# ivanalberico/End-To-End-Self-Supervised-SLAM

Hardware: AMD Instinct MI355X
Metric: online refinement steps/sec @640x480, seq_len=60 (higher is better)
Workload: dtype f32

## Files before the change

### end-to-end-self-supervised-slam_amd/csrc/conv.hip

```cpp
#include <cassert>
#include <type_traits>

#include "e2e_common.h"

typedef float f4v __attribute__((ext_vector_type(4)));
typedef float f16v __attribute__((ext_vector_type(16)));

#define CBK 16

enum { ACT_NONE = 0, ACT_RELU = 1, ACT_ELU = 2, ACT_DISP = 3 };

struct ConvArgs {
    const float* src0;
    const float* src1;
    const float* w;
    const float* scale;
    const float* shift;
    const float* res;
    float* out;
    int B, Hs, Ws;
    int Cin, C1, up;
    int Hd, Wd;
    int Ncols, ldw;
    int KH, KW, stride, pad, pad_mode;
// ... 794 lines not shown
#pragma unroll
            for (int q = 0; q < 4; ++q) {
                const f4v t = {v[4 * q], v[4 * q + 1], v[4 * q + 2], v[4 * q + 3]};
                __builtin_amdgcn_raw_buffer_store_b128(__builtin_bit_cast(__attribute__((__vector_size__(4 * sizeof(unsigned)))) unsigned, t), rsl, sl_off + q * 64 * 16, 0, SK_SC1);
            }
            asm volatile("s_waitcnt vmcnt(0)" ::: "memory");
            __syncthreads();
            if (tid == 0) __hip_atomic_store(&s.flags[g], 1u, __ATOMIC_RELAXED, __HIP_MEMORY_SCOPE_AGENT);
        } else {
            if (ce != s.C) {
                const int64_t tile_end = (int64_t)(tile + 1) * s.C;
                int h_last = g;
                for (int h = g + 1; h < s.G && s.I * h / s.G < tile_end; ++h) h_last = h;
                if (tid == 0) {
                    for (int h = g + 1; h <= h_last; ++h) {
                        unsigned spins = 0;
                        while (__hip_atomic_load(&s.flags[h], __ATOMIC_RELAXED, __HIP_MEMORY_SCOPE_AGENT) == 0u) {
                            __builtin_amdgcn_s_sleep(2);
                            if (++spins > (1u << 24)) { __hip_atomic_store(&s.flags[SK_ERR_INDEX], 1u, __ATOMIC_RELAXED, __HIP_MEMORY_SCOPE_AGENT); break; }
                        }
                    }
                    __builtin_amdgcn_fence(__ATOMIC_ACQUIRE, "agent");
                }
                asm volatile("s_waitcnt vmcnt(0)" ::: "memory");
                __syncthreads();
                for (int h = g + 1; h <= h_last; ++h) {
                    const __amdgpu_buffer_rsrc_t rsl = __builtin_amdgcn_make_buffer_rsrc((void*)(s.slabs + (int64_t)h * (BM * BN)), 0, BM * BN * 4, 0x00020000);
                    f4v t[4];
#pragma unroll
                    for (int q = 0; q < 4; ++q) t[q] = __builtin_bit_cast(f4v, __builtin_amdgcn_raw_buffer_load_b128(rsl, sl_off + q * 64 * 16, 0, SK_SC1));
#pragma unroll
                    for (int q = 0; q < 4; ++q)
#pragma unroll
                        for (int e = 0; e < 4; ++e) acc[4 * q + e] += t[q][e];
                }
                if (tid == 0)
                    for (int h = g + 1; h <= h_last; ++h) __hip_atomic_store(&s.flags[h], 0u, __ATOMIC_RELAXED, __HIP_MEMORY_SCOPE_AGENT);
            }
            const EpiRsrc er = make_epi_rsrc<TRANSPOSED>(a);
            epilogue_block<TRANSPOSED>(a, er, acc, c0 + wn * 32 + (lane & 31), n0 + wm * 32 + 4 * khalf, Ntot);
        }
        it += ce - cb;
    }
}

struct ThinArgs {
    const float* src;
    const float* w;
    const float* bias;
    float* out;
    int B, Hsrc, Wsrc, Hd, Wd, ldw, act, org, flip;
};

template <int CIN, int UP, bool REFLECT, int TH>
__global__ __launch_bounds__(256) void k_conv3x3_thin(ThinArgs a) {
    constexpr int TW = 64, PH = TH + 2, PW = TW + 2, PWS = 72, PLANE = PH * PWS, KQ = CIN / 4;
    static_assert(PLANE % 32 == 16, "the two channel planes a half-wave reads must sit 16 banks apart");
    __shared__ float patch[CIN * PLANE];
    const int tid = threadIdx.x, lane = tid & 63, wave = tid >> 6, l16 = lane & 15, kq = lane >> 4;
    const int x0 = blockIdx.x * TW, y0 = blockIdx.y * TH, b = blockIdx.z;
    const int HD = a.Hsrc * UP, WD = a.Wsrc * UP;
    float wreg[9][KQ];
#pragma unroll
    for (int t = 0; t < 9; ++t)
#pragma unroll
        for (int j = 0; j < KQ; ++j) wreg[t][j] = a.w[(int64_t)((a.flip ? 8 - t : t) * CIN + 4 * j + kq) * a.ldw + l16];
    const float* sb = a.src + (int64_t)b * a.Hsrc * a.Wsrc * CIN;
    for (int idx = tid; idx < PH * PW * KQ; idx += 256) {
        const int q = (UP == 2) ? idx / (PH * PW) : idx % KQ, pix = (UP == 2) ? idx % (PH * PW) : idx / KQ;
        const int py = pix / PW, px = pix - py * PW;
        int Y = y0 - a.org + py, X = x0 - a.org + px;
        bool ok = true;
        if (REFLECT) {
            Y = min(max(reflect1(Y, HD), 0), HD - 1);
            X = min(max(reflect1(X, WD), 0), WD - 1);
        } else {
            ok = Y >= 0 && Y < HD && X >= 0 && X < WD;
        }
        f4v v = {0.f, 0.f, 0.f, 0.f};
        if (ok) v = *(const f4v*)(sb + ((int64_t)(Y / UP) * a.Wsrc + (X / UP)) * CIN + q * 4);
#pragma unroll
        for (int e = 0; e < 4; ++e) patch[(q * 4 + e) * PLANE + py * PWS + px] = v[e];
    }
    __syncthreads();
    const float bv = a.bias ? a.bias[l16] : 0.f;
    float* ob = a.out + (int64_t)b * a.Hd * a.Wd * 16;
#pragma unroll 1
    for (int g2 = 0; g2 < TH; g2 += 2) {
        const int g0 = wave * TH + g2, g1 = g0 + 1;
        const int r0 = g0 >> 2, c0 = (g0 & 3) * 16, r1 = g1 >> 2, c1 = (g1 & 3) * 16;
        f4v acc0 = {0.f, 0.f, 0.f, 0.f}, acc1 = {0.f, 0.f, 0.f, 0.f};
        const float* p0 = patch + kq * PLANE + r0 * PWS + c0 + l16;
        const float* p1 = patch + kq * PLANE + r1 * PWS + c1 + l16;
#pragma unroll
        for (int t = 0; t < 9; ++t) {
            const int off = (t / 3) * PWS + (t % 3);
#pragma unroll
            for (int j = 0; j < KQ; ++j) {
                acc0 = __builtin_amdgcn_mfma_f32_16x16x4f32(p0[4 * j * PLANE + off], wreg[t][j], acc0, 0, 0, 0);
                acc1 = __builtin_amdgcn_mfma_f32_16x16x4f32(p1[4 * j * PLANE + off], wreg[t][j], acc1, 0, 0, 0);
            }
        }
#pragma unroll
        for (int h = 0; h < 2; ++h) {
            const f4v acc = h ? acc1 : acc0;
            const int y = y0 + (h ? r1 : r0), xb = x0 + (h ? c1 : c0) + 4 * kq;
            if (y >= a.Hd) continue;
#pragma unroll
            for (int i = 0; i < 4; ++i)
                if (xb + i < a.Wd) ob[((int64_t)y * a.Wd + xb + i) * 16 + l16] = apply_act(acc[i] + bv, a.act);
        }
    }
}

struct StemArgs {
    const float* src;
    const float* w;
    const float* scale;
    const float* shift;
    float* out;
    int B, Hs, Ws, Hd, Wd, ldw, act;
    float in_sub, in_mul;
};

__global__ __launch_bounds__(256) void k_conv7x7_stem(StemArgs a) {
    constexpr int TH = 4, TW = 32, PH = 2 * TH + 6, PW = 2 * TW + 5, ROW = 208, NJ = 37;
    __shared__ float patch[PH * ROW];
    const int tid = threadIdx.x, lane = tid & 63, wave = tid >> 6, l16 = lane & 15, kq = lane >> 4;
    const int x0 = blockIdx.x * TW, y0 = blockIdx.y * TH, b = blockIdx.z;
    const int co = 16 * wave + l16;
    float wreg[NJ];
    int offk[NJ];
#pragma unroll
    for (int j = 0; j < NJ; ++j) {
        const int k = 4 * j + kq;
        wreg[j] = k < 147 ? a.w[(int64_t)k * a.ldw + co] : 0.f;
        offk[j] = k + (k / 21) * (ROW - 21);
    }
    const float* sb = a.src + (int64_t)b * a.Hs * a.Ws * 3;
    for (int idx = tid; idx < PH * ROW; idx += 256) {
        const int py = idx / ROW, e = idx - py * ROW;
        const int Y = 2 * y0 - 3 + py, X = 2 * x0 - 3 + e / 3;
        const bool ok = e < 3 * PW && Y >= 0 && Y < a.Hs && X >= 0 && X < a.Ws;
        patch[idx] = ok ? (sb[((int64_t)Y * a.Ws + X) * 3 + (e - (e / 3) * 3)] - a.in_sub) * a.in_mul : 0.f;
    }
    __syncthreads();
    const float sc = a.scale ? a.scale[co] : 1.f, sh = a.shift ? a.shift[co] : 0.f;
    float* ob = a.out + (int64_t)b * a.Hd * a.Wd * 64;
#pragma unroll 1
    for (int g = 0; g < 2 * TH; g += 2) {
        const int r = g >> 1;
        const float* p0 = patch + 2 * r * ROW + 6 * l16;
        const float* p1 = p0 + 6 * 16;
        f4v acc0 = {0.f, 0.f, 0.f, 0.f}, acc1 = {0.f, 0.f, 0.f, 0.f};
#pragma unroll
        for (int j = 0; j < NJ; ++j) {
            acc0 = __builtin_amdgcn_mfma_f32_16x16x4f32(p0[offk[j]], wreg[j], acc0, 0, 0, 0);
            acc1 = __builtin_amdgcn_mfma_f32_16x16x4f32(p1[offk[j]], wreg[j], acc1, 0, 0, 0);
        }
        const int y = y0 + r;
        if (y >= a.Hd) continue;
#pragma unroll
        for (int h = 0; h < 2; ++h) {
            const f4v acc = h ? acc1 : acc0;
            const int xb = x0 + 16 * h + 4 * kq;
// ... 903 lines not shown
    __shared__ float dzs[TH * TW * 64];
    const int tid = threadIdx.x, lane = tid & 63, wave = tid >> 6, l16 = lane & 15, kq = lane >> 4;
    const int y0 = blockIdx.y * TH, b = blockIdx.z;
    int offn[10];
#pragma unroll
    for (int nt = 0; nt < 10; ++nt) {
        const int k = 16 * nt + l16;
        offn[nt] = k + (k / 21) * (ROW - 21) + 48 * kq;
    }
    f4v acc[10];
#pragma unroll
    for (int nt = 0; nt < 10; ++nt) acc[nt] = (f4v){0.f, 0.f, 0.f, 0.f};
    const float* sb = a.src + (int64_t)b * a.Hs * a.Ws * 3;
    const float* zb = a.dz + (int64_t)b * a.Hd * a.Wd * 64;
    for (int tx = 0; tx < a.tiles_x; ++tx) {
        const int x0 = (blockIdx.x * a.tiles_x + tx) * TW;
        if (x0 >= a.Wd) break;
        __syncthreads();
        for (int idx = tid; idx < PH * ROW; idx += 256) {
            const int py = idx / ROW, e = idx - py * ROW;
            const int Y = 2 * y0 - 3 + py, X = 2 * x0 - 3 + e / 3;
            const bool ok = e < 3 * PW && Y >= 0 && Y < a.Hs && X >= 0 && X < a.Ws;
            patch[idx] = ok ? (sb[((int64_t)Y * a.Ws + X) * 3 + (e - (e / 3) * 3)] - a.in_sub) * a.in_mul : 0.f;
        }
        for (int idx = tid; idx < TH * TW * 16; idx += 256) {
            const int q = idx & 15, pix = idx >> 4;
            const int r = pix / TW, x = pix - r * TW;
            const bool ok = y0 + r < a.Hd && x0 + x < a.Wd;
            *(f4v*)&dzs[pix * 64 + q * 4] = ok ? *(const f4v*)(zb + ((int64_t)(y0 + r) * a.Wd + x0 + x) * 64 + q * 4) : (f4v){0.f, 0.f, 0.f, 0.f};
        }
        __syncthreads();
#pragma unroll 1
        for (int r = 0; r < TH; ++r) {
            const float* ap = dzs + (r * TW + 8 * kq) * 64 + 16 * wave + l16;
            const float* bp = patch + 2 * r * ROW;
#pragma unroll 2
            for (int ks = 0; ks < TW / 4; ++ks) {
                const float av = ap[ks * 64];
#pragma unroll
                for (int nt = 0; nt < 10; ++nt) acc[nt] = __builtin_amdgcn_mfma_f32_16x16x4f32(av, bp[offn[nt] + ks * 6], acc[nt], 0, 0, 0);
            }
        }
    }
    float* slab = a.slabs + (((int64_t)b * gridDim.y + blockIdx.y) * a.nxg + blockIdx.x) * 64 * NPAD;
#pragma unroll
    for (int nt = 0; nt < 10; ++nt)
#pragma unroll
        for (int i = 0; i < 4; ++i) {
            const int n = 16 * nt + l16;
            if (n < 147) slab[(16 * wave + 4 * kq + i) * NPAD + n] = acc[nt][i];
        }
}

struct TapWgradArgs {
    const float* dz;
    const float* src0;
    const float* src1;
    float* slabs;
    int B, H, W, Cin, C1, up, Cout, reflect, has_bias, Mpad, Npad;
    int ptx, pty;
    int nchunks, cps;
};

#define TAP_NT 192
template <bool BIAS>
__global__ __launch_bounds__(TAP_NT) void k_wgrad3x3_taps(TapWgradArgs a) {
    __shared__ float dzs[64 * 32];
    __shared__ float xs[100 * 32];
    const int tid = threadIdx.x, lane = tid & 63, wave = tid >> 6, kh_ = lane >> 5, l32 = lane & 31;
    const int ci0 = blockIdx.x * 32, co0 = blockIdx.y * 32;
    const bool first = ci0 < a.C1;
    const int sh = first ? (a.up >> 1) : 0, Cs = first ? a.C1 : a.Cin - a.C1, cs0 = first ? ci0 : ci0 - a.C1;
    const int Hs = a.H >> sh, Ws = a.W >> sh;
    const float* sbase = first ? a.src0 : a.src1;
    const int c_begin = blockIdx.z * a.cps, c_end = min(c_begin + a.cps, a.nchunks);
    const bool want_bias = BIAS && blockIdx.x == 0 && wave == 0;
    f16v acc[3], accb;
#pragma unroll
    for (int t = 0; t < 3; ++t)
#pragma unroll
        for (int r = 0; r < 16; ++r) acc[t][r] = 0.f;
#pragma unroll
    for (int r = 0; r < 16; ++r) accb[r] = 0.f;
    const float one = (l32 == 0) ? 1.f : 0.f;
    f4v rz[3], rx[5];
    auto load_chunk = [&](int g) {
        const int b = g / (a.pty * a.ptx), rem = g - b * (a.pty * a.ptx), py = rem / a.ptx, px = rem - py * a.ptx;
        const int y0 = py * 8, x0 = px * 8;
        const float* zb = a.dz + (int64_t)b * a.H * a.W * a.Cout + co0;
        const float* sb = sbase + (int64_t)b * Hs * Ws * Cs + cs0;
#pragma unroll
        for (int i = 0; i < 3; ++i) {
            const int f = tid + TAP_NT * i, pix = f >> 3, q = f & 7, y = y0 + (pix >> 3), x = x0 + (pix & 7);
            const bool ok = f < 512 && y < a.H && x < a.W;
            rz[i] = ok ? *(const f4v*)(zb + ((int64_t)y * a.W + x) * a.Cout + q * 4) : (f4v){0.f, 0.f, 0.f, 0.f};
        }
#pragma unroll
        for (int i = 0; i < 5; ++i) {
            const int f = tid + TAP_NT * i;
            f4v v = {0.f, 0.f, 0.f, 0.f};
            if (f < 800) {
                const int pix = f >> 3, q = f & 7;
                int y = y0 - 1 + pix / 10, x = x0 - 1 + pix % 10;
                bool ok = true;
                if (a.reflect) {
                    y = min(max(reflect1(y, a.H), 0), a.H - 1);
// ... 857 lines not shown
    return E2E_OK;
}

struct ConvGeom { int B, Hs, Ws, Cin, Cout, Ho, Wo, KH, KW, stride, pad, pad_mode, C1, up; float in_sub, in_mul; };
#define GEOM_LAYER(g) ConvGeom g{}; g.B = B; g.Hs = Hs; g.Ws = Ws; g.Cin = Cin; g.Cout = Cout; g.KH = KH; g.KW = KW; g.stride = stride; g.pad = pad; g.pad_mode = pad_mode
#define GEOM_SOURCES(g) g.C1 = C1; g.up = up; g.in_sub = in_sub; g.in_mul = in_mul
#define GEOM_OUTPUT(g) g.Ho = Ho; g.Wo = Wo
#define GEOM_BWD_DATA(g) GEOM_LAYER(g); GEOM_OUTPUT(g)
#define GEOM_BWD_WEIGHT(g) GEOM_LAYER(g); GEOM_OUTPUT(g); GEOM_SOURCES(g)
#define GEOM_WGRAD_QUERY(g) ConvGeom g{}; g.B = B; g.Ho = Ho; g.Wo = Wo; g.Cin = Cin; g.Cout = Cout; g.KH = KH; g.KW = KW
struct FwdOps { const float *src0, *src1, *w_fwd; int ld_fwd; const float *scale, *shift, *residual; float* out; int act; };
struct BwdDataOps { const float* dz; const float* w_bwd; int ld_bwd; float* dxp; int accumulate; const float* x_in; int in_act; const float* pre_add; };
struct WgradIn { const float *dz, *src0, *src1; float* workspace; };

static int fwd_setup(const FwdOps& f, const ConvGeom& g, ConvArgs& a_out, int& vec_out, const char* who) {
    const int B = g.B, Hs = g.Hs, Ws = g.Ws, Cin = g.Cin, Cout = g.Cout, KH = g.KH, KW = g.KW, stride = g.stride, pad = g.pad, pad_mode = g.pad_mode;
    const int C1 = g.C1, up = g.up, ld_fwd = f.ld_fwd;
    E2E_REQUIRE(f.src0 && f.w_fwd && f.out && B > 0 && Hs > 0 && Ws > 0 && Cin > 0 && Cout > 0 && KH > 0 && KW > 0, E2E_ERR_ARG, "%s: bad argument", who);
    E2E_REQUIRE(up == 1 || up == 2, E2E_ERR_ARG, "%s: upsample factor must be 1 or 2", who);
    E2E_REQUIRE(C1 > 0 && C1 <= Cin && (C1 == Cin || f.src1), E2E_ERR_ARG, "%s: bad channel split", who);
    E2E_REQUIRE(pad_mode == 0 || (pad_mode == 1 && pad == 1 && Hs >= 2 && Ws >= 2), E2E_ERR_ARG, "%s: reflection padding needs pad == 1", who);
    E2E_REQUIRE(stride == 1 || stride == 2, E2E_ERR_ARG, "%s: stride must be 1 or 2", who);
    E2E_REQUIRE(Hs % up == 0 && Ws % up == 0 && ld_fwd % 4 == 0 && ld_fwd >= Cout, E2E_ERR_ARG, "%s: bad sizes", who);
    E2E_REQUIRE(pad >= 0 && Hs + 2 * pad >= KH && Ws + 2 * pad >= KW, E2E_ERR_ARG, "%s: the kernel must fit the padded input (pad >= 0)", who);
    const int vec = (Cin % 16 == 0 && (C1 == Cin || C1 % 16 == 0)) ? 4 : 1;
    E2E_REQUIRE(vec == 4 || (C1 == Cin && up == 1), E2E_ERR_ARG, "%s: the scalar path (Cin %% 16 != 0) takes a single full-resolution source", who);
    E2E_REQUIRE((int64_t)B * Hs * Ws * Cin * 4 < (1ll << 30) && (int64_t)KH * KW * Cin * ld_fwd * 4 < (1ll << 31), E2E_ERR_ARG,
                "%s: activations must stay below 1 GB, weights below 2 GB (32-bit buffer offsets with out-of-range markers)", who);
    E2E_REQUIRE(vec != 4 || (KH <= 3 && KW <= 3), E2E_ERR_ARG, "%s: the channel-quad loader takes kernels up to 3 x 3", who);
    ConvArgs a{};
    a.src0 = f.src0; a.src1 = f.src1; a.w = f.w_fwd; a.scale = f.scale; a.shift = f.shift; a.res = f.residual; a.out = f.out;
    a.B = B; a.Hs = Hs; a.Ws = Ws; a.Cin = Cin; a.C1 = C1; a.up = up;
    a.Hd = (Hs + 2 * pad - KH) / stride + 1; a.Wd = (Ws + 2 * pad - KW) / stride + 1;
    a.Ncols = Cout; a.ldw = ld_fwd; a.KH = KH; a.KW = KW; a.stride = stride; a.pad = pad; a.pad_mode = pad_mode; a.off = 0; a.act = f.act;
    a.in_sub = g.in_sub; a.in_mul = g.in_mul;
    a_out = a; vec_out = vec;
    return E2E_OK;
}

static int conv_fwd_impl(const FwdOps& f, const ConvGeom& g, float* workspace, GemmCfg force, void* stream) {
    const int B = g.B, Hs = g.Hs, Ws = g.Ws, Cin = g.Cin, Cout = g.Cout, KH = g.KH, KW = g.KW, stride = g.stride, pad = g.pad, pad_mode = g.pad_mode;
    const int C1 = g.C1, up = g.up, ld_fwd = f.ld_fwd;
    ConvArgs a;
    int vec;
    const int rc = fwd_setup(f, g, a, vec, "e2e_conv2d_fwd");
    if (rc != E2E_OK) return rc;
    if (!force.bm && KH == 7 && KW == 7 && stride == 2 && pad == 3 && pad_mode == 0 && Cin == 3 && Cout == 64 && C1 == Cin && up == 1 && !f.residual && ld_fwd >= 64) {
        StemArgs t{f.src0, f.w_fwd, f.scale, f.shift, f.out, B, Hs, Ws, a.Hd, a.Wd, ld_fwd, f.act, g.in_sub, g.in_mul};
        hipLaunchKernelGGL(k_conv7x7_stem, dim3((a.Wd + 31) / 32, (a.Hd + 3) / 4, B), dim3(256), 0, (hipStream_t)stream, t);
    }
    else if (!force.bm && KH == 3 && KW == 3 && stride == 1 && pad == 1 && pad_mode == 1 && Cout == 16 && C1 == Cin && !f.scale && !f.residual && ld_fwd >= 16 &&
        ((Cin == 16 && up == 2) || (Cin == 32 && up == 1))) {
        ThinArgs t{f.src0, f.w_fwd, f.shift, f.out, B, Hs / up, Ws / up, Hs, Ws, ld_fwd, f.act, 1, 0};
        if (Cin == 16) hipLaunchKernelGGL((k_conv3x3_thin<16, 2, true, 8>), dim3((Ws + 63) / 64, (Hs + 7) / 8, B), dim3(256), 0, (hipStream_t)stream, t);
        else hipLaunchKernelGGL((k_conv3x3_thin<32, 1, true, 4>), dim3((Ws + 63) / 64, (Hs + 3) / 4, B), dim3(256), 0, (hipStream_t)stream, t);
    } else
        launch_gemm<false>(a, vec, workspace, force, (hipStream_t)stream);
    E2E_LAUNCH_CHECK("e2e_conv2d_fwd");
    return E2E_OK;
}

int e2e_conv2d_fwd(const float* src0, const float* src1, int C1, int up, const float* w_fwd, int ld_fwd, const float* scale,
                   const float* shift, const float* residual, float* out, int B, int Hs, int Ws, int Cin, int Cout, int KH,
                   int KW, int stride, int pad, int pad_mode, int act, float in_sub, float in_mul, float* workspace, void* stream) {
    GEOM_LAYER(g); GEOM_SOURCES(g);
    return conv_fwd_impl(FwdOps{src0, src1, w_fwd, ld_fwd, scale, shift, residual, out, act}, g, workspace, GemmCfg{0, 0, 0}, stream);
}

static bool tuning_ok(int tile_m, int tile_n, int ksplit) {
    if (tile_m == 0) return true;
    if (ksplit < 0) return tile_m == 64 && tile_n == 64 && -ksplit <= SK_MAX_G;
    return tile_max_cb(tile_m, tile_n) != 0 && ksplit >= 1 && ksplit <= 16;
}

int e2e_conv2d_fwd_tuned(const float* src0, const float* src1, int C1, int up, const float* w_fwd, int ld_fwd, const float* scale,
                         const float* shift, const float* residual, float* out, int B, int Hs, int Ws, int Cin, int Cout, int KH,
                         int KW, int stride, int pad, int pad_mode, int act, float in_sub, float in_mul, float* workspace, int tile_m, int tile_n,
                         int ksplit, void* stream) {
    E2E_REQUIRE(tuning_ok(tile_m, tile_n, ksplit), E2E_ERR_ARG, "e2e_conv2d_fwd_tuned: unsupported decomposition %d x %d / %d", tile_m, tile_n, ksplit);
    GEOM_LAYER(g); GEOM_SOURCES(g);
    return conv_fwd_impl(FwdOps{src0, src1, w_fwd, ld_fwd, scale, shift, residual, out, act}, g, workspace, GemmCfg{tile_m, tile_n, ksplit}, stream);
}

struct EntryOps {
    const float* x;
    const float *w1_fwd; int ld1; const float *scale1, *shift1; float* out1; int act1; float* workspace1;
    const float* wd_fwd; int ldd; const float *gamma, *beta, *mean, *var; float eps; float *bn_scale, *bn_shift, *bn_rstd, *z, *y;
};
struct EntryPlan { ConvArgs a1, ad; int vec1, vecd; GemmLaunch p1, pd; ConvGeom g1, gd; bool paired; };

static int fwd_entry_plan(const EntryOps& q, const ConvGeom& g, EntryPlan& P, const char* who) {
    E2E_REQUIRE(q.gamma && q.beta && q.mean && q.var && q.bn_scale && q.bn_shift && q.bn_rstd && q.z && q.y, E2E_ERR_ARG, "%s: bad argument", who);
    E2E_REQUIRE(g.pad_mode == 0 && g.C1 == g.Cin && g.up == 1, E2E_ERR_ARG, "%s: a stage entry reads one zero-padded full-resolution source", who);
    P.g1 = g;
    P.gd = g; P.gd.KH = P.gd.KW = 1; P.gd.pad = 0;
    int rc = fwd_setup(FwdOps{q.x, nullptr, q.w1_fwd, q.ld1, q.scale1, q.shift1, nullptr, q.out1, q.act1}, P.g1, P.a1, P.vec1, who);
    if (rc != E2E_OK) return rc;
    rc = fwd_setup(FwdOps{q.x, nullptr, q.wd_fwd, q.ldd, nullptr, nullptr, nullptr, q.z, ACT_NONE}, P.gd, P.ad, P.vecd, who);
    if (rc != E2E_OK) return rc;
    E2E_REQUIRE(P.a1.Hd == P.ad.Hd && P.a1.Wd == P.ad.Wd, E2E_ERR_ARG, "%s: the two branches must produce the same output grid", who);
    P.paired = false;
    if (P.vec1 != 4 || P.vecd != 4 || g.Cout < 128) return E2E_OK;
    P.p1 = plan_gemm<false>(P.a1, 4, q.workspace1, GemmCfg{0, 0, 0});
    P.pd = plan_gemm<false>(P.ad, 4, nullptr, GemmCfg{0, 0, 0});
    auto t14 = [](const GemmLaunch& p) { return p.kind == GK_TILE && p.cb == 32 && p.c.bm == 32 && p.c.bn == 128; };
    P.paired = t14(P.p1) && t14(P.pd) && P.pd.tail == GT_NONE && P.ad.ksplit == 1 && P.pd.g.z == 1;
    return E2E_OK;
}
// ... 5 lines not shown
    const int pad_mode = 0, C1 = Cin, up = 1;
    const float in_sub = 0.f, in_mul = 1.f;
    GEOM_LAYER(g); GEOM_SOURCES(g);
    const EntryOps q{x, w1_fwd, ld1, scale1, shift1, out1, act1, workspace1, wd_fwd, ldd, gamma, beta, running_mean, running_var, eps, bn_scale, bn_shift, bn_rstd, z, y};
    EntryPlan P;
    int rc = fwd_entry_plan(q, g, P, "e2e_conv2d_fwd_entry_pair");
    if (rc != E2E_OK) return rc;
    const hipStream_t st = (hipStream_t)stream;
    if (!P.paired) {
        rc = conv_fwd_impl(FwdOps{x, nullptr, w1_fwd, ld1, scale1, shift1, nullptr, out1, act1}, P.g1, workspace1, GemmCfg{0, 0, 0}, stream);
        if (rc != E2E_OK) return rc;
        rc = conv_fwd_impl(FwdOps{x, nullptr, wd_fwd, ldd, nullptr, nullptr, nullptr, z, ACT_NONE}, P.gd, nullptr, GemmCfg{0, 0, 0}, stream);
        if (rc != E2E_OK) return rc;
        rc = e2e_bn_fold(gamma, beta, running_mean, running_var, eps, bn_scale, bn_shift, bn_rstd, Cout, stream);
        if (rc != E2E_OK) return rc;
        return e2e_affine_fwd(z, bn_scale, bn_shift, nullptr, 0, y, (int64_t)B * P.ad.Hd * P.ad.Wd * Cout, Cout, stream);
    }
    FwdPairGrid pg;
    pg.agx = P.p1.g.x; pg.agy = P.p1.g.y; pg.agz = P.p1.g.z;
    pg.bgx = P.pd.g.x; pg.bgy = P.pd.g.y;
    pg.first = (pg.agx * pg.agy * pg.agz + 7u) / 8u * 8u;
    const BnFoldArgs bn{gamma, beta, running_mean, running_var, eps, bn_scale, bn_shift, bn_rstd, y};
    hipLaunchKernelGGL(k_conv_fwd_pair, dim3(pg.first + pg.bgx * pg.bgy), dim3(256), 0, st, P.a1, P.ad, bn, pg);
    launch_gemm_tail(P.a1, P.p1, st);
    E2E_LAUNCH_CHECK("e2e_conv2d_fwd_entry_pair");
    return E2E_OK;
}

int e2e_conv2d_fwd_entry_pair_is_one_launch(int ld1, int ldd, int has_workspace1, int B, int Hs, int Ws, int Cin, int Cout, int KH, int KW, int stride, int pad) {
    static float nowhere[4];
    float* const p = nowhere;
    const int pad_mode = 0, C1 = Cin, up = 1;
    const float in_sub = 0.f, in_mul = 1.f;
    GEOM_LAYER(g); GEOM_SOURCES(g);
    const EntryOps q{p, p, ld1, p, p, p, ACT_RELU, has_workspace1 ? p : nullptr, p, ldd, p, p, p, p, 0.f, p, p, p, p, p};
    EntryPlan P;
    if (fwd_entry_plan(q, g, P, "e2e_conv2d_fwd_entry_pair_is_one_launch") != E2E_OK) return 0;
    return P.paired ? 1 : 0;
}

static int bwd_data_setup(const BwdDataOps& d, const ConvGeom& g, GemmCfg force, hipStream_t stream, ConvArgs& a, bool& done, bool dry = false) {
    const int B = g.B, Hs = g.Hs, Ws = g.Ws, Cin = g.Cin, Cout = g.Cout, Ho = g.Ho, Wo = g.Wo, KH = g.KH, KW = g.KW, stride = g.stride, pad = g.pad;
    const int pad_mode = g.pad_mode, ld_bwd = d.ld_bwd;
    done = false;
    E2E_REQUIRE(d.pre_add == nullptr || pad_mode == 0, E2E_ERR_ARG, "e2e_conv2d_bwd_data: the pre-activation addend takes a zero-padded layer");
    E2E_REQUIRE(d.in_act == 0 || (d.x_in && (d.in_act == ACT_RELU || d.in_act == ACT_ELU) && pad_mode == 0), E2E_ERR_ARG,
                "e2e_conv2d_bwd_data: the fused input-activation derivative takes ReLU / ELU, the activation's output and a zero-padded layer");
    E2E_REQUIRE(d.dz && d.w_bwd && d.dxp && B > 0 && Cin > 0 && Cout > 0 && Cout % 16 == 0, E2E_ERR_ARG, "e2e_conv2d_bwd_data: bad argument (Cout %% 16 == 0)");
    E2E_REQUIRE(ld_bwd % 4 == 0 && ld_bwd >= Cin && (stride == 1 || stride == 2), E2E_ERR_ARG, "e2e_conv2d_bwd_data: bad sizes");
    E2E_REQUIRE((int64_t)B * Ho * Wo * Cout * 4 < (1ll << 30) && (int64_t)KH * KW * Cout * ld_bwd * 4 < (1ll << 31) && KH <= 3 && KW <= 3, E2E_ERR_ARG,
                "e2e_conv2d_bwd_data: gradients must stay below 1 GB, weights below 2 GB (32-bit buffer offsets), kernels up to 3 x 3");
    if (!force.bm && KH == 3 && KW == 3 && stride == 1 && pad == 1 && pad_mode == 1 && Cin == 16 && Cout == 16 && !d.accumulate && !d.in_act && !d.pre_add && ld_bwd >= 16) {
        ThinArgs t{d.dz, d.w_bwd, nullptr, d.dxp, B, Ho, Wo, Hs + 2, Ws + 2, ld_bwd, ACT_NONE, 2, 1};
        if (!dry) hipLaunchKernelGGL((k_conv3x3_thin<16, 1, false, 8>), dim3((Ws + 2 + 63) / 64, (Hs + 2 + 7) / 8, B), dim3(256), 0, stream, t);
        done = true;
        return E2E_OK;
    }
    a = ConvArgs{};
    a.src0 = d.dz; a.src1 = nullptr; a.w = d.w_bwd; a.out = d.dxp;
    a.B = B; a.Hs = Ho; a.Ws = Wo; a.Cin = Cout; a.C1 = Cout; a.up = 1;
    const int pp = pad_mode == 1 ? pad : 0;
    a.Hd = Hs + 2 * pp; a.Wd = Ws + 2 * pp; a.off = pad_mode == 1 ? 0 : pad;
    a.Ncols = Cin; a.ldw = ld_bwd; a.KH = KH; a.KW = KW; a.stride = stride; a.pad = pad; a.pad_mode = 0; a.act = ACT_NONE;
    a.cls = (stride == 2 && cls_rows(B, a.Hd, a.Wd) < (1 << 24)) ? 1 : 0;
    if (a.cls && (KH < 2 || KW < 2) && !d.accumulate && !dry)
        (void)hipMemsetAsync(d.dxp, 0, (size_t)B * a.Hd * a.Wd * Cin * sizeof(float), stream);
    if (d.accumulate) a.res = d.dxp;
    a.xin = d.in_act ? d.x_in : nullptr; a.dact = d.in_act; a.pre = d.pre_add;
    return E2E_OK;
}

static int bwd_data_impl(const BwdDataOps& d, const ConvGeom& g, float* workspace, void* stream, GemmCfg force = GemmCfg{0, 0, 0}) {
    ConvArgs a;
    bool done;
    const int rc = bwd_data_setup(d, g, force, (hipStream_t)stream, a, done);
    if (rc != E2E_OK) return rc;
    if (!done) launch_gemm<true>(a, 4, workspace, force, (hipStream_t)stream);
    E2E_LAUNCH_CHECK("e2e_conv2d_bwd_data");
    return E2E_OK;
}

int e2e_conv2d_bwd_data(const float* dz, const float* w_bwd, int ld_bwd, float* dxp, int B, int Hs, int Ws, int Cin, int Cout,
                        int Ho, int Wo, int KH, int KW, int stride, int pad, int pad_mode, float* workspace, void* stream) {
    GEOM_BWD_DATA(g);
    return bwd_data_impl(BwdDataOps{dz, w_bwd, ld_bwd, dxp, 0, nullptr, 0, nullptr}, g, workspace, stream);
}

int e2e_conv2d_bwd_data_acc(const float* dz, const float* w_bwd, int ld_bwd, float* dxp, int B, int Hs, int Ws, int Cin, int Cout,
                            int Ho, int Wo, int KH, int KW, int stride, int pad, int pad_mode, int accumulate, float* workspace,
                            void* stream) {
    GEOM_BWD_DATA(g);
    return bwd_data_impl(BwdDataOps{dz, w_bwd, ld_bwd, dxp, accumulate, nullptr, 0, nullptr}, g, workspace, stream);
}

int e2e_conv2d_bwd_data_fused(const float* da, const float* w_bwd, int ld_bwd, float* dxp, int B, int Hs, int Ws, int Cin, int Cout,
                              int Ho, int Wo, int KH, int KW, int stride, int pad, int pad_mode, int accumulate, const float* x_in,
                              int in_act, const float* pre_add, float* workspace, void* stream) {
    GEOM_BWD_DATA(g);
    return bwd_data_impl(BwdDataOps{da, w_bwd, ld_bwd, dxp, accumulate, x_in, in_act, pre_add}, g, workspace, stream);
}

int e2e_conv2d_bwd_data_fused_tuned(const float* da, const float* w_bwd, int ld_bwd, float* dxp, int B, int Hs, int Ws, int Cin, int Cout,
                                    int Ho, int Wo, int KH, int KW, int stride, int pad, int pad_mode, int accumulate, const float* x_in,
                                    int in_act, const float* pre_add, float* workspace, int tile_m, int tile_n, int ksplit, void* stream) {
    E2E_REQUIRE(tuning_ok(tile_m, tile_n, ksplit), E2E_ERR_ARG, "e2e_conv2d_bwd_data_fused_tuned: unsupported decomposition %d x %d / %d", tile_m, tile_n, ksplit);
    GEOM_BWD_DATA(g);
    return bwd_data_impl(BwdDataOps{da, w_bwd, ld_bwd, dxp, accumulate, x_in, in_act, pre_add}, g, workspace, stream, GemmCfg{tile_m, tile_n, ksplit});
// ... 148 lines not shown
        (p = plan(WP_STEM)).open)
        return p;
    if (lean && stride == 1 && pad == 1 && pad_mode == 1 && C1 % 16 == 0 && Ho == Hs && Wo == Ws && (C1 == Cin || has_src1) && Hs % up == 0 && Ws % up == 0 &&
        (p = plan(WP_THIN)).open)
        return p;
    if (vec == 4 && stride == 1 && pad == 1 && Ho == Hs && Wo == Ws && (up == 1 || up == 2) && Hs % up == 0 && Ws % up == 0 && (C1 == Cin || (has_src1 && C1 % 32 == 0)) &&
        getenv("E2E_WGRAD_TAPS") != nullptr && getenv("E2E_WGRAD_TAPS")[0] == '1' && (p = plan(WP_TAPS)).open)
        return p;
    return lean && (p = plan(WP_GEMM16)).open ? p : plan(lean ? WP_GEMM_LEAN : WP_GEMM);
}

int64_t e2e_conv2d_wgrad_workspace_floats(int B, int Ho, int Wo, int Cin, int Cout, int KH, int KW, int has_bias) {
    GEOM_WGRAD_QUERY(g);
    return wgrad_workspace_floats(g, has_bias, false, WGRAD_TARGET);
}

struct WgradOut { float* dw; float* dbias; const float* out_scale; int accumulate; e2e_wgrad_reduce_desc* defer; };

static void wgrad_reduce(const WgradArgs& a, const WgradOut& o, int S, int Mpad, int Npad, int zl, hipStream_t st) {
    if (o.defer) {
        *o.defer = e2e_wgrad_reduce_desc{a.slabs, o.dw, o.dbias, o.out_scale, S, Mpad, Npad, a.Cout, a.Cin, a.KH, a.KW, a.has_bias, o.accumulate, zl, 0};
        return;
    }
    const int64_t tq = (int64_t)a.Cout * ((a.Ngemm + 3) / 4);
    if (zl == 8)
        hipLaunchKernelGGL((k_wgrad_reduce<8>), dim3(egrid(tq * 4)), dim3(512), 0, st, a.slabs, S, Mpad, Npad, a.Cout, a.Cin, a.KH, a.KW, a.has_bias, o.dw,
                           o.dbias, o.accumulate, o.out_scale);
    else
        hipLaunchKernelGGL((k_wgrad_reduce<2>), dim3(egrid(tq * 4)), dim3(128), 0, st, a.slabs, S, Mpad, Npad, a.Cout, a.Cin, a.KH, a.KW, a.has_bias, o.dw,
                           o.dbias, o.accumulate, o.out_scale);
}

enum WgradKernel { WK_DONE, WK_GEMM16, WK_GEMM4_32, WK_GEMM4_64, WK_GEMM_32, WK_GEMM_64 };
struct WgradLaunch { WgradKernel k; dim3 g; int Sz; };

static int wgrad_setup(const WgradIn& in, const ConvGeom& g, int wg_target, const WgradOut& o, hipStream_t st, WgradArgs& a, WgradLaunch& L, bool dry = false) {
    const int B = g.B, Cin = g.Cin, Cout = g.Cout, Ho = g.Ho, Wo = g.Wo;
    const bool tuned = wg_target != 0;
    if (!tuned) wg_target = WGRAD_TARGET;
    L = WgradLaunch{WK_DONE, dim3(1), 0};
    E2E_REQUIRE(in.dz && in.src0 && o.dw && in.workspace && B > 0 && Cin > 0 && Cout > 0, E2E_ERR_ARG, "e2e_conv2d_bwd_weight: bad argument");
    const int vec = (Cin % 4 == 0 && g.C1 % 4 == 0) ? 4 : 1;
    E2E_REQUIRE(vec == 4 || (g.C1 == Cin && g.up == 1 && g.pad_mode == 0), E2E_ERR_ARG, "e2e_conv2d_bwd_weight: scalar path takes one full-resolution zero-padded source");
    a = WgradArgs{};
    a.dz = in.dz; a.src0 = in.src0; a.src1 = in.src1; a.slabs = in.workspace;
    a.B = B; a.Hs = g.Hs; a.Ws = g.Ws; a.Cin = Cin; a.C1 = g.C1; a.up = g.up; a.Ho = Ho; a.Wo = Wo; a.Cout = Cout;
    a.KH = g.KH; a.KW = g.KW; a.stride = g.stride; a.pad = g.pad; a.pad_mode = g.pad_mode; a.has_bias = o.dbias ? 1 : 0;
    a.Ngemm = g.KH * g.KW * Cin + a.has_bias;
    const WgradPlan p = wgrad_choose(g, a.has_bias, in.src1 != nullptr, tuned, wg_target);
    const int S = (int)p.S;
    if (dry && (p.path == WP_STEM || p.path == WP_THIN || p.path == WP_TAPS)) return E2E_OK;
    if (p.path == WP_STEM) {
        StemWgradArgs ta{in.dz, in.src0, in.workspace, B, g.Hs, g.Ws, Ho, Wo, 2, p.nxg, g.in_sub, g.in_mul};
        hipLaunchKernelGGL(k_wgrad7x7_stem, dim3(p.nxg, p.ny, B), dim3(256), 0, st, ta);
    } else if (p.path == WP_THIN) {
        ThinWgradArgs ta{in.dz, in.src0, in.src1, in.workspace, B, Ho, Wo, Cin, g.C1, g.up, p.Npad, a.has_bias, p.tiles_x, p.nxg};
        const dim3 tg((unsigned)p.nxg, (unsigned)p.ny, (unsigned)(B * (Cin / 16)));
        const char* ev = getenv("E2E_THIN_WGRAD_REGS");
        const bool regs = !(ev && ev[0] == '0') && (int64_t)Wo * Cout * 4 < (1ll << 31);
        if (regs && Cout == 32) hipLaunchKernelGGL((k_wgrad3x3_thin_regs<2>), tg, dim3(256), 0, st, ta);
        else if (regs) hipLaunchKernelGGL((k_wgrad3x3_thin_regs<1>), tg, dim3(256), 0, st, ta);
        else if (Cout == 32) hipLaunchKernelGGL((k_wgrad3x3_thin<2>), tg, dim3(256), 0, st, ta);
        else hipLaunchKernelGGL((k_wgrad3x3_thin<1>), tg, dim3(256), 0, st, ta);
    } else if (p.path == WP_TAPS) {
        TapWgradArgs ta{in.dz, in.src0, in.src1, in.workspace, B, Ho, Wo, Cin, g.C1, g.up, Cout, g.pad_mode == 1 ? 1 : 0, a.has_bias,
                        p.Mpad, p.Npad, p.ptx, p.pty, p.nchunks, p.cps};
        const dim3 tg((unsigned)(Cin / 32), (unsigned)(Cout / 32), (unsigned)S);
        if (a.has_bias) hipLaunchKernelGGL(k_wgrad3x3_taps<true>, tg, dim3(TAP_NT), 0, st, ta);
        else hipLaunchKernelGGL(k_wgrad3x3_taps<false>, tg, dim3(TAP_NT), 0, st, ta);
    }
    if (p.path == WP_STEM || p.path == WP_THIN || p.path == WP_TAPS) {
        wgrad_reduce(a, o, S, p.Mpad, p.Npad, (p.path == WP_TAPS && S < 8) ? 2 : 8, st);
        return E2E_OK;
    }
    const bool use16 = p.path == WP_GEMM16, lean = p.path != WP_GEMM;
    a.Mpad = p.Mpad; a.Npad = p.Npad;
    a.in_sub = g.in_sub; a.in_mul = g.in_mul; a.vec = vec;
    const int64_t P = (int64_t)B * Ho * Wo;
    const int cbp = lean ? 32 : CBK;
    a.pix_per_slice = ((P + p.S - 1) / p.S + cbp - 1) / cbp * cbp;
    L.Sz = (int)((P + a.pix_per_slice - 1) / a.pix_per_slice);
    L.g = dim3((unsigned)(a.Npad / p.tn), (unsigned)(a.Mpad / p.tm), (unsigned)L.Sz);
    L.k = use16 ? WK_GEMM16 : lean ? (p.tm == 32 ? WK_GEMM4_32 : WK_GEMM4_64) : (p.tm == 32 ? WK_GEMM_32 : WK_GEMM_64);
    return E2E_OK;
}

static void wgrad_launch_gemm(const WgradArgs& a, const WgradLaunch& L, hipStream_t st) {
    const dim3 g = L.g;
    const bool two = a.src1 != nullptr;
    if (L.k == WK_GEMM16) hipLaunchKernelGGL((k_wgrad_gemm16<10, 32>), g, dim3(256), 0, st, a);
    else if (L.k == WK_GEMM4_32 && two) hipLaunchKernelGGL((k_wgrad_gemm4<1, 4, 32, true>), g, dim3(256), 0, st, a);
    else if (L.k == WK_GEMM4_32) hipLaunchKernelGGL((k_wgrad_gemm4<1, 4, 32, false>), g, dim3(256), 0, st, a);
    else if (L.k == WK_GEMM4_64 && two) hipLaunchKernelGGL((k_wgrad_gemm4<2, 2, 32, true>), g, dim3(256), 0, st, a);
    else if (L.k == WK_GEMM4_64) hipLaunchKernelGGL((k_wgrad_gemm4<2, 2, 32, false>), g, dim3(256), 0, st, a);
    else if (L.k == WK_GEMM_32 && a.vec == 4) hipLaunchKernelGGL((k_wgrad_gemm<1, 4, 4>), g, dim3(256), 0, st, a);
    else if (L.k == WK_GEMM_32) hipLaunchKernelGGL((k_wgrad_gemm<1, 4, 1>), g, dim3(256), 0, st, a);
    else if (L.k == WK_GEMM_64 && a.vec == 4) hipLaunchKernelGGL((k_wgrad_gemm<2, 2, 4>), g, dim3(256), 0, st, a);
    else if (L.k == WK_GEMM_64) hipLaunchKernelGGL((k_wgrad_gemm<2, 2, 1>), g, dim3(256), 0, st, a);
}

static int bwd_weight_impl(const WgradIn& in, const ConvGeom& g, const WgradOut& o, void* stream, int wg_target = 0) {
    const hipStream_t st = (hipStream_t)stream;
    WgradArgs a;
    WgradLaunch L;
    const int rc = wgrad_setup(in, g, wg_target, o, st, a, L);
    if (rc != E2E_OK) return rc;
    if (L.k != WK_DONE) {
// ... 183 lines not shown
```

Measured before the change: 225.5.

## Add retiled thin 3x3 conv kernels and register-staged stem weight-gradient kernel

Generalizes the thin 3x3 conv kernel over tile width and adds a variant that stages the x2 nearest-upsampled input at source resolution in shared memory, then indexes it directly, instead of replicating pixels. New smaller-tile launches with waves-per-EU hints are used by default for the forward Cin=16 and Cin=32 paths and for the backward-data thin path. A stem 7x7 weight-gradient kernel now preloads dz into registers before staging the patch. All four new paths are on by default with environment switches to disable them, and they trade larger grids and register pressure for less staging work and higher occupancy.

Result: no change. 227.1 (median of 6 runs) (+0.7%).

```diff
diff --git a/end-to-end-self-supervised-slam_amd/csrc/conv.hip b/end-to-end-self-supervised-slam_amd/csrc/conv.hip
--- a/end-to-end-self-supervised-slam_amd/csrc/conv.hip
+++ b/end-to-end-self-supervised-slam_amd/csrc/conv.hip
@@ -870,10 +870,19 @@
     int B, Hsrc, Wsrc, Hd, Wd, ldw, act, org, flip;
 };
 
-template <int CIN, int UP, bool REFLECT, int TH>
-__global__ __launch_bounds__(256) void k_conv3x3_thin(ThinArgs a) {
-    constexpr int TW = 64, PH = TH + 2, PW = TW + 2, PWS = 72, PLANE = PH * PWS, KQ = CIN / 4;
-    static_assert(PLANE % 32 == 16, "the two channel planes a half-wave reads must sit 16 banks apart");
+constexpr int thin_row_stride(int ph, int pw) {
+    for (int s = pw; s < pw + 32; ++s)
+        if ((ph * s) % 32 == 16) return s;
+    return 0;
+}
+
+template <int CIN, int UP, bool REFLECT, int TH, int TW, bool SRC>
+__device__ __forceinline__ void conv3x3_thin_body(const ThinArgs& a) {
+    static_assert(!SRC || (UP == 2 && REFLECT && TH % 2 == 0), "source-resolution staging serves the reflection-padded x2 upsample");
+    constexpr int GW = TW / 16, GPW = TH * GW / 4;
+    static_assert(TW % 16 == 0 && (TH * GW) % 8 == 0, "every wave sweeps an even number of 16-pixel groups");
+    constexpr int PH = SRC ? TH / 2 + 2 : TH + 2, PW = SRC ? TW / 2 + 2 : TW + 2, PWS = thin_row_stride(PH, PW), PLANE = PH * PWS, KQ = CIN / 4;
+    static_assert(PWS != 0 && PLANE % 32 == 16, "the two channel planes a half-wave reads must sit 16 banks apart");
     __shared__ float patch[CIN * PLANE];
     const int tid = threadIdx.x, lane = tid & 63, wave = tid >> 6, l16 = lane & 15, kq = lane >> 4;
     const int x0 = blockIdx.x * TW, y0 = blockIdx.y * TH, b = blockIdx.z;
@@ -885,18 +894,24 @@
         for (int j = 0; j < KQ; ++j) wreg[t][j] = a.w[(int64_t)((a.flip ? 8 - t : t) * CIN + 4 * j + kq) * a.ldw + l16];
     const float* sb = a.src + (int64_t)b * a.Hsrc * a.Wsrc * CIN;
     for (int idx = tid; idx < PH * PW * KQ; idx += 256) {
-        const int q = (UP == 2) ? idx / (PH * PW) : idx % KQ, pix = (UP == 2) ? idx % (PH * PW) : idx / KQ;
+        constexpr bool PIXFAST = UP == 2 && !SRC;
+        const int q = PIXFAST ? idx / (PH * PW) : idx % KQ, pix = PIXFAST ? idx % (PH * PW) : idx / KQ;
         const int py = pix / PW, px = pix - py * PW;
-        int Y = y0 - a.org + py, X = x0 - a.org + px;
-        bool ok = true;
-        if (REFLECT) {
-            Y = min(max(reflect1(Y, HD), 0), HD - 1);
-            X = min(max(reflect1(X, WD), 0), WD - 1);
+        f4v v = {0.f, 0.f, 0.f, 0.f};
+        if (SRC) {
+            const int Y = min(max((y0 >> 1) - 1 + py, 0), a.Hsrc - 1), X = min(max((x0 >> 1) - 1 + px, 0), a.Wsrc - 1);
+            v = *(const f4v*)(sb + ((int64_t)Y * a.Wsrc + X) * CIN + q * 4);
         } else {
-            ok = Y >= 0 && Y < HD && X >= 0 && X < WD;
-        }
-        f4v v = {0.f, 0.f, 0.f, 0.f};
-        if (ok) v = *(const f4v*)(sb + ((int64_t)(Y / UP) * a.Wsrc + (X / UP)) * CIN + q * 4);
+            int Y = y0 - a.org + py, X = x0 - a.org + px;
+            bool ok = true;
+            if (REFLECT) {
+                Y = min(max(reflect1(Y, HD), 0), HD - 1);
+                X = min(max(reflect1(X, WD), 0), WD - 1);
+            } else {
+                ok = Y >= 0 && Y < HD && X >= 0 && X < WD;
+            }
+            if (ok) v = *(const f4v*)(sb + ((int64_t)(Y / UP) * a.Wsrc + (X / UP)) * CIN + q * 4);
+        }
 #pragma unroll
         for (int e = 0; e < 4; ++e) patch[(q * 4 + e) * PLANE + py * PWS + px] = v[e];
     }
@@ -904,19 +919,35 @@
     const float bv = a.bias ? a.bias[l16] : 0.f;
     float* ob = a.out + (int64_t)b * a.Hd * a.Wd * 16;
 #pragma unroll 1
-    for (int g2 = 0; g2 < TH; g2 += 2) {
-        const int g0 = wave * TH + g2, g1 = g0 + 1;
-        const int r0 = g0 >> 2, c0 = (g0 & 3) * 16, r1 = g1 >> 2, c1 = (g1 & 3) * 16;
+    for (int g2 = 0; g2 < GPW; g2 += 2) {
+        const int g0 = wave * GPW + g2, g1 = g0 + 1;
+        const int r0 = g0 / GW, c0 = (g0 % GW) * 16, r1 = g1 / GW, c1 = (g1 % GW) * 16;
         f4v acc0 = {0.f, 0.f, 0.f, 0.f}, acc1 = {0.f, 0.f, 0.f, 0.f};
-        const float* p0 = patch + kq * PLANE + r0 * PWS + c0 + l16;
-        const float* p1 = patch + kq * PLANE + r1 * PWS + c1 + l16;
-#pragma unroll
-        for (int t = 0; t < 9; ++t) {
-            const int off = (t / 3) * PWS + (t % 3);
-#pragma unroll
-            for (int j = 0; j < KQ; ++j) {
-                acc0 = __builtin_amdgcn_mfma_f32_16x16x4f32(p0[4 * j * PLANE + off], wreg[t][j], acc0, 0, 0, 0);
-                acc1 = __builtin_amdgcn_mfma_f32_16x16x4f32(p1[4 * j * PLANE + off], wreg[t][j], acc1, 0, 0, 0);
+        if (SRC) {
+            const float* q0 = patch + kq * PLANE + ((c0 + l16 + 1) >> 1);
+            const float* q1 = patch + kq * PLANE + ((c1 + l16 + 1) >> 1);
+            const int mid = (l16 + 1) & 1;
+#pragma unroll
+            for (int t = 0; t < 9; ++t) {
+                const int kh = t / 3, kw = t % 3;
+                const int o0 = ((r0 + 1 + kh) >> 1) * PWS + (kw == 1 ? mid : kw >> 1), o1 = ((r1 + 1 + kh) >> 1) * PWS + (kw == 1 ? mid : kw >> 1);
+#pragma unroll
+                for (int j = 0; j < KQ; ++j) {
+                    acc0 = __builtin_amdgcn_mfma_f32_16x16x4f32(q0[4 * j * PLANE + o0], wreg[t][j], acc0, 0, 0, 0);
+                    acc1 = __builtin_amdgcn_mfma_f32_16x16x4f32(q1[4 * j * PLANE + o1], wreg[t][j], acc1, 0, 0, 0);
+                }
+            }
+        } else {
+            const float* p0 = patch + kq * PLANE + r0 * PWS + c0 + l16;
+            const float* p1 = patch + kq * PLANE + r1 * PWS + c1 + l16;
+#pragma unroll
+            for (int t = 0; t < 9; ++t) {
+                const int off = (t / 3) * PWS + (t % 3);
+#pragma unroll
+                for (int j = 0; j < KQ; ++j) {
+                    acc0 = __builtin_amdgcn_mfma_f32_16x16x4f32(p0[4 * j * PLANE + off], wreg[t][j], acc0, 0, 0, 0);
+                    acc1 = __builtin_amdgcn_mfma_f32_16x16x4f32(p1[4 * j * PLANE + off], wreg[t][j], acc1, 0, 0, 0);
+                }
             }
         }
 #pragma unroll
@@ -929,6 +960,24 @@
                 if (xb + i < a.Wd) ob[((int64_t)y * a.Wd + xb + i) * 16 + l16] = apply_act(acc[i] + bv, a.act);
         }
     }
+}
+
+template <int CIN, int UP, bool REFLECT, int TH>
+__global__ __launch_bounds__(256) void k_conv3x3_thin(ThinArgs a) {
+    conv3x3_thin_body<CIN, UP, REFLECT, TH, 64, false>(a);
+}
+
+template <int CIN, int UP, bool REFLECT, int TH, int TW, bool SRC, int WPE>
+__global__ __launch_bounds__(256) __attribute__((amdgpu_waves_per_eu(WPE))) void k_conv3x3_thin_tile(ThinArgs a) {
+    conv3x3_thin_body<CIN, UP, REFLECT, TH, TW, SRC>(a);
+}
+template <int CIN, int UP, bool REFLECT, int TH, int TW, bool SRC, int WPE>
+static void launch_thin_tile(const ThinArgs& t, hipStream_t st) {
+    hipLaunchKernelGGL((k_conv3x3_thin_tile<CIN, UP, REFLECT, TH, TW, SRC, WPE>), dim3((t.Wd + TW - 1) / TW, (t.Hd + TH - 1) / TH, t.B), dim3(256), 0, st, t);
+}
+static bool switch_on(const char* name) {
+    const char* ev = getenv(name);
+    return !(ev && ev[0] == '0');
 }
 
 struct StemArgs {
@@ -1938,6 +1987,60 @@
         }
 }
 
+__global__ __launch_bounds__(256) __attribute__((amdgpu_waves_per_eu(4))) void k_wgrad7x7_stem_regs(StemWgradArgs a) {
+    constexpr int TH = 4, TW = 32, PH = 2 * TH + 6, PW = 2 * TW + 5, ROW = 208, NPAD = 148;
+    __shared__ float patch[PH * ROW];
+    const int tid = threadIdx.x, lane = tid & 63, wave = tid >> 6, l16 = lane & 15, kq = lane >> 4;
+    const int y0 = blockIdx.y * TH, b = blockIdx.z;
+    int offn[10];
+#pragma unroll
+    for (int nt = 0; nt < 10; ++nt) {
+        const int k = 16 * nt + l16;
+        offn[nt] = k + (k / 21) * (ROW - 21) + 48 * kq;
+    }
+    f4v acc[10];
+#pragma unroll
+    for (int nt = 0; nt < 10; ++nt) acc[nt] = (f4v){0.f, 0.f, 0.f, 0.f};
+    const float* sb = a.src + (int64_t)b * a.Hs * a.Ws * 3;
+    const float* zb = a.dz + (int64_t)b * a.Hd * a.Wd * 64 + 16 * wave + l16;
+    for (int tx = 0; tx < a.tiles_x; ++tx) {
+        const int x0 = (blockIdx.x * a.tiles_x + tx) * TW;
+        if (x0 >= a.Wd) break;
+        float av[TH][TW / 4];
+#pragma unroll
+        for (int r = 0; r < TH; ++r)
+#pragma unroll
+            for (int ks = 0; ks < TW / 4; ++ks) {
+                const int y = y0 + r, x = x0 + ks + 8 * kq;
+                av[r][ks] = (y < a.Hd && x < a.Wd) ? zb[((int64_t)y * a.Wd + x) * 64] : 0.f;
+            }
+        __syncthreads();
+        for (int idx = tid; idx < PH * ROW; idx += 256) {
+            const int py = idx / ROW, e = idx - py * ROW;
+            const int Y = 2 * y0 - 3 + py, X = 2 * x0 - 3 + e / 3;
+            const bool ok = e < 3 * PW && Y >= 0 && Y < a.Hs && X >= 0 && X < a.Ws;
+            patch[idx] = ok ? (sb[((int64_t)Y * a.Ws + X) * 3 + (e - (e / 3) * 3)] - a.in_sub) * a.in_mul : 0.f;
+        }
+        __syncthreads();
+#pragma unroll
+        for (int r = 0; r < TH; ++r) {
+            const float* bp = patch + 2 * r * ROW;
+#pragma unroll
+            for (int ks = 0; ks < TW / 4; ++ks)
+#pragma unroll
+                for (int nt = 0; nt < 10; ++nt) acc[nt] = __builtin_amdgcn_mfma_f32_16x16x4f32(av[r][ks], bp[offn[nt] + ks * 6], acc[nt], 0, 0, 0);
+        }
+    }
+    float* slab = a.slabs + (((int64_t)b * gridDim.y + blockIdx.y) * a.nxg + blockIdx.x) * 64 * NPAD;
+#pragma unroll
+    for (int nt = 0; nt < 10; ++nt)
+#pragma unroll
+        for (int i = 0; i < 4; ++i) {
+            const int n = 16 * nt + l16;
+            if (n < 147) slab[(16 * wave + 4 * kq + i) * NPAD + n] = acc[nt][i];
+        }
+}
+
 struct TapWgradArgs {
     const float* dz;
     const float* src0;
@@ -2901,8 +3004,11 @@
     else if (!force.bm && KH == 3 && KW == 3 && stride == 1 && pad == 1 && pad_mode == 1 && Cout == 16 && C1 == Cin && !f.scale && !f.residual && ld_fwd >= 16 &&
         ((Cin == 16 && up == 2) || (Cin == 32 && up == 1))) {
         ThinArgs t{f.src0, f.w_fwd, f.shift, f.out, B, Hs / up, Ws / up, Hs, Ws, ld_fwd, f.act, 1, 0};
-        if (Cin == 16) hipLaunchKernelGGL((k_conv3x3_thin<16, 2, true, 8>), dim3((Ws + 63) / 64, (Hs + 7) / 8, B), dim3(256), 0, (hipStream_t)stream, t);
-        else hipLaunchKernelGGL((k_conv3x3_thin<32, 1, true, 4>), dim3((Ws + 63) / 64, (Hs + 3) / 4, B), dim3(256), 0, (hipStream_t)stream, t);
+        hipStream_t st = (hipStream_t)stream;
+        if (Cin == 16 && switch_on("E2E_THIN_FWD_SRCRES")) launch_thin_tile<16, 2, true, 8, 16, true, 5>(t, st);
+        else if (Cin == 16) hipLaunchKernelGGL((k_conv3x3_thin<16, 2, true, 8>), dim3((Ws + 63) / 64, (Hs + 7) / 8, B), dim3(256), 0, st, t);
+        else if (switch_on("E2E_THIN32_TILE")) launch_thin_tile<32, 1, true, 8, 16, false, 3>(t, st);
+        else hipLaunchKernelGGL((k_conv3x3_thin<32, 1, true, 4>), dim3((Ws + 63) / 64, (Hs + 3) / 4, B), dim3(256), 0, st, t);
     } else
         launch_gemm<false>(a, vec, workspace, force, (hipStream_t)stream);
     E2E_LAUNCH_CHECK("e2e_conv2d_fwd");
@@ -3014,7 +3120,9 @@
                 "e2e_conv2d_bwd_data: gradients must stay below 1 GB, weights below 2 GB (32-bit buffer offsets), kernels up to 3 x 3");
     if (!force.bm && KH == 3 && KW == 3 && stride == 1 && pad == 1 && pad_mode == 1 && Cin == 16 && Cout == 16 && !d.accumulate && !d.in_act && !d.pre_add && ld_bwd >= 16) {
         ThinArgs t{d.dz, d.w_bwd, nullptr, d.dxp, B, Ho, Wo, Hs + 2, Ws + 2, ld_bwd, ACT_NONE, 2, 1};
-        if (!dry) hipLaunchKernelGGL((k_conv3x3_thin<16, 1, false, 8>), dim3((Ws + 2 + 63) / 64, (Hs + 2 + 7) / 8, B), dim3(256), 0, stream, t);
+        if (dry) ;
+        else if (switch_on("E2E_THIN_BWD_TILE")) launch_thin_tile<16, 1, false, 4, 32, false, 8>(t, stream);
+        else hipLaunchKernelGGL((k_conv3x3_thin<16, 1, false, 8>), dim3((Ws + 2 + 63) / 64, (Hs + 2 + 7) / 8, B), dim3(256), 0, stream, t);
         done = true;
         return E2E_OK;
     }
@@ -3269,7 +3377,8 @@
     if (dry && (p.path == WP_STEM || p.path == WP_THIN || p.path == WP_TAPS)) return E2E_OK;
     if (p.path == WP_STEM) {
         StemWgradArgs ta{in.dz, in.src0, in.workspace, B, g.Hs, g.Ws, Ho, Wo, 2, p.nxg, g.in_sub, g.in_mul};
-        hipLaunchKernelGGL(k_wgrad7x7_stem, dim3(p.nxg, p.ny, B), dim3(256), 0, st, ta);
+        if (switch_on("E2E_STEM_WGRAD_TILE")) hipLaunchKernelGGL(k_wgrad7x7_stem_regs, dim3(p.nxg, p.ny, B), dim3(256), 0, st, ta);
+        else hipLaunchKernelGGL(k_wgrad7x7_stem, dim3(p.nxg, p.ny, B), dim3(256), 0, st, ta);
     } else if (p.path == WP_THIN) {
         ThinWgradArgs ta{in.dz, in.src0, in.src1, in.workspace, B, Ho, Wo, Cin, g.C1, g.up, p.Npad, a.has_bias, p.tiles_x, p.nxg};
         const dim3 tg((unsigned)p.nxg, (unsigned)p.ny, (unsigned)(B * (Cin / 16)));
```
